# fraunhoferhhi/casapose

Measured on AMD Instinct MI355X. Metric: images/sec at 640x480, 8-object LMO (casapose_c_gcu5 forward + component filter + LS keypoint voting), higher is better.
Workload: dtype f32 (fp32-level: every fp32 operand as an fp16 pair hi = rn(x), lo = rn(x - hi) -- reproduced to within one fp32 ulp, 0.75 x 2^-24 rms -- and the three products hi*hi, hi*lo, lo*hi, each exact, accumulated in fp32 on v_mfma_f32_32x32x16_f16; weights pre-scaled by a power of two; measured error again; 1 GPU; config_8.ini inference: casapose_c_gcu5, K=9 classes, ver_dim=27, bs=16 per GPU, 480x640, fp32, estimated-mask conditioning, connected-component filter + LS voting; conv_mode=f16x2, parallelism=replicas x1 (no collective)

## Files before the change

### casapose_amd/_lib.py

```python
from __future__ import annotations

import ctypes as C
import os
from typing import Optional

import torch

_HERE = os.path.dirname(os.path.abspath(__file__))
LIB_PATH = os.environ.get("CASAPOSE_HIP_LIB") or os.path.join(_HERE, "libcasapose_hip.so")


class CasaposeHipError(RuntimeError):
    pass


class ConvSource(C.Structure):
    _fields_ = [
        ("data", C.c_void_p),
        ("channels", C.c_int),
        ("ld", C.c_int),
        ("mode", C.c_int),
        ("sel", C.c_void_p),
        ("pre_scale", C.c_void_p),
        ("pre_shift", C.c_void_p),
# ... 93 lines not shown

_vp, _i, _ll, _f = C.c_void_p, C.c_int, C.c_longlong, C.c_float
SYMBOLS = [
    ("cp_last_error", C.c_char_p, []),
    ("cp_version", _i, []),
    ("cp_conv_desc_size", C.c_size_t, []),
    ("cp_conv_source_size", C.c_size_t, []),
    ("cp_device_count", _i, []),
    ("cp_set_persistent_blocks", _i, [_i]),
    ("cp_get_persistent_blocks", _i, []),
    ("cp_mfma_probe_workspace_bytes", C.c_size_t, []),
    ("cp_mfma_probe", _i, [_i, _i, _vp, C.POINTER(C.c_double), _vp]),
    ("cp_conv_ktot", _i, [_i, _i, _i, C.POINTER(_i)]),
    ("cp_conv_pack_weights_host", _i, [_vp, _i, _i, _i, _i, _i, C.POINTER(_i), C.POINTER(_i), _vp]),
    ("cp_conv_halo_weight_floats", _i, [_i, _i, C.POINTER(_i)]),
    ("cp_conv_pack_weights_halo_host", _i, [_vp, _i, _i, _i, C.POINTER(_i), C.POINTER(_i), _vp]),
    ("cp_conv_pack_weights_stem_host", _i, [_vp, _i, _i, _vp]),
    ("cp_conv_pack_head_weights_host", _i, [_vp, _i, _vp]),
    ("cp_conv2d_fwd_f32", _i, [C.POINTER(ConvDesc), _vp]),
    ("cp_conv_selected_tile", _i, [C.POINTER(ConvDesc)]),
    ("cp_conv_split_applicable", _i, [C.POINTER(ConvDesc)]),
    ("cp_conv_split_weight_floats", _i, [_i, _i, C.POINTER(_i)]),
    ("cp_conv_split_weight_bytes", C.c_size_t, [_i, _i, C.POINTER(_i), _i]),
    ("cp_conv_pack_weights_split_host", _i, [_vp, _i, _i, _i, C.POINTER(_i), C.POINTER(_i), _vp]),
    ("cp_conv_split_weights_f32", _i, [_vp, _ll, _i, _vp, _vp]),
    ("cp_conv_pack_head_split_host", _i, [_vp, _i, _vp]),
    ("cp_conv2d_fwd_split", _i, [C.POINTER(ConvDesc), _vp, _vp, _i, _vp]),
    ("cp_conv_split_weights_scaled_f32", _i, [_vp, _ll, _i, C.c_float, _vp, _vp]),
    ("cp_conv2d_fwd_split_scaled", _i, [C.POINTER(ConvDesc), _vp, _vp, _i, C.c_float, C.c_float, _vp]),
    ("cp_conv_bf16_deep_applicable", _i, [C.POINTER(ConvDesc)]),
    ("cp_conv2d_fwd_bf16_deep", _i, [C.POINTER(ConvDesc), _vp, _vp]),
    ("cp_pad_channels_3to4", _i, [_vp, _vp, _ll, _vp]),
    ("cp_maxpool3x3s2_f32", _i, [_vp, _i, _i, _i, _i, _vp, _vp, _i, _vp, _vp]),
    ("cp_upsample_bilinear_x2_f32", _i, [_vp, _i, _i, _i, _i, _vp, _vp]),
    ("cp_guided_upsample_x2_f32", _i, [_vp, _vp, _i, _i, _i, _i, _vp, _vp]),
    ("cp_mask_to_labels_f32", _i, [_vp, _i, _i, _i, _i, _vp, _vp, _vp]),
    ("cp_argmax_labels", _i, [_vp, _i, _i, _ll, _vp, _vp]),
    ("cp_label_pyramid", _i, [_vp, _i, _i, _i, C.POINTER(_vp), C.POINTER(_vp), C.POINTER(_vp), _vp]),
    ("cp_ls_vote_f32", _i, [_vp, _i, _i, _i, _i, _vp, _i, _i, _i, _i, _i, _vp, _vp, _vp]),
    ("cp_ls_vote_w_f32", _i, [_vp, _i, _i, _i, _i, _vp, _i, _i, _i, _i, _i, _i, _vp, _vp, _vp]),
    ("cp_ls_vote_workspace_bytes", C.c_size_t, [_i, _i, _i]),
    ("cp_ccl_filter_labels", _i, [_vp, _i, _i, _i, _i, _i, _i, _vp, _vp, _vp]),
    ("cp_ccl_workspace_bytes", C.c_size_t, [_i, _i, _i, _i]),
    ("cp_ransac_vote_f32", _i, [_vp, _vp, _i, _i, _i, _i, _i, _i, _i, _vp, _i, _f, _f, _i, _i, _i, _vp, _vp, _vp, _vp]),
    ("cp_ransac_vote_seeded_f32", _i, [_vp, _vp, _i, _i, _i, _i, _i, _i, _i, C.c_ulonglong, _i, _f, _f, _i, _i, _i, _vp, _vp, _vp, _vp]),
    ("cp_ransac_workspace_bytes", C.c_size_t, [_i, _i, _i, _i, _i, _i]),
# ... 117 lines not shown
```

### casapose_amd/csrc/conv_hsplit.hip

```cpp
#include "common.h"
#include "mfma_helpers.h"

#include <algorithm>
#include <cmath>
#include <cstdlib>
#include <type_traits>

namespace {

using namespace cp;

constexpr int COLS = 34;
constexpr int TH = 8;
constexpr int HR = TH + 2;
constexpr int HP = HR * COLS;
constexpr int PLANE_B = HP * 32;
constexpr int IPLANE_B = HP * 8;
constexpr int NIT = (HP * 4 + 255) / 256;
constexpr int NIMG = (HP + 255) / 256;

enum : int { HS_BILINEAR = 2, HS_PARTIAL = 4, HS_SEL = 8, HS_HEADK = 16, HS_PREFIX = 32 };

struct SSrc {
    const float* data;
    const uint8_t* sel;
    int C, ld, Hs, Ws;
    unsigned bytes;
};

struct HSplitK {
    SSrc s[2];
    const float* img;
    unsigned img_bytes;
    const unsigned char* W;
    unsigned w_bytes;
    int B, H, Wd, Cout;
    int nch0, nch;
    int tiles_y, tiles_x, ntiles;
    int passes, tiles_per_pass;
    const uint8_t* label;
    unsigned lab_bytes;
    const float* residual;
    int res_ld;
    const float* scale;
// ... 85 lines not shown
            *reinterpret_cast<uint4*>(d + 2048) = make_uint4(l0.x, l0.y, l1.x, l1.y);
        } else if constexpr (NP == 2) {
            uint2 h0, l0, h1, l1;
            cp::split4h(make_float4(v0.x * scale, v0.y * scale, v0.z * scale, v0.w * scale), h0, l0);
            cp::split4h(make_float4(v1.x * scale, v1.y * scale, v1.z * scale, v1.w * scale), h1, l1);
            *reinterpret_cast<uint4*>(d) = make_uint4(h0.x, h0.y, h1.x, h1.y);
            *reinterpret_cast<uint4*>(d + 1024) = make_uint4(l0.x, l0.y, l1.x, l1.y);
        } else {
            const uint2 a = round4(v0), b = round4(v1);
            *reinterpret_cast<uint4*>(d) = make_uint4(a.x, a.y, b.x, b.y);
        }
    }
}

__device__ __forceinline__ float leaky01(float t) { return fmaxf(t, 0.1f * t); }

#ifdef HS_GT3
__host__ __device__ constexpr int hs_group_taps(int tn, int np) { return tn == 1 ? 9 : (tn == 2 ? 3 : 1); }
#else
__host__ __device__ constexpr int hs_group_taps(int tn, int np) { return tn == 1 ? 9 : (tn == 2 ? (np <= 2 ? 9 : 3) : 1); }
#endif

template <int TN, int NP, int MODE>
__global__ __launch_bounds__(512, 2) void conv_hsplit_kernel(const HSplitK p) {
    constexpr bool PARTIAL = (MODE & HS_PARTIAL) != 0;
    constexpr bool BILINEAR = (MODE & HS_BILINEAR) != 0;
    constexpr bool SEL = (MODE & HS_SEL) != 0;
    constexpr bool HEADK = (MODE & HS_HEADK) != 0;
    constexpr bool PREFIX = (MODE & HS_PREFIX) != 0;
    static_assert(!PREFIX || HEADK, "only head layers write output records");
    static_assert(!HEADK || TN == 1, "a fused head needs 32 output channels");
    constexpr int NV = 1;
    constexpr unsigned OOB = 0x80000000u;
    static_assert(NP == 1 || NP == 2 || NP == 3, "1 = bf16, 2 = fp16 two-way split, 3 = exact bf16 split");
    constexpr int NPROD = (NP == 3) ? 6 : (NP == 2) ? 3 : 1;
    constexpr unsigned FRAG_B = NP * 1024u;
    constexpr int GT = hs_group_taps(TN, NP);
    constexpr int GPS = 9 / GT;
    constexpr int GSUB = GT * TN;
    constexpr unsigned GROUP_B = GSUB * FRAG_B;
    constexpr unsigned IGROUP_B = 3 * TN * FRAG_B;
    static_assert(TN == 1 || TN == 2 || TN == 4, "32, 64 or 128 output channels per pass");
    constexpr int NWL = (int)((GROUP_B / 16 + 255) / 256);

    const bool has_img = p.img != nullptr;
    extern __shared__ __attribute__((aligned(16))) unsigned char smem[];
    unsigned char* halo = smem;
    unsigned char* imgh = smem + 2 * NP * PLANE_B;
    unsigned short* labh = reinterpret_cast<unsigned short*>(smem + 2 * NP * PLANE_B + 2 * NP * IPLANE_B);
    unsigned char* wst = smem + 2 * NP * PLANE_B + 2 * NP * IPLANE_B + 4 * HP;
    unsigned char* hwl = wst + ((HEADK && NP <= 2) ? 2 * GROUP_B + IGROUP_B : 2 * GROUP_B);
    constexpr int LOW_R = HR / 2 + 1, LOW_C = COLS / 2 + 1, LOW_P = LOW_R * LOW_C;
    constexpr int LOW_B = LOW_P * 64;
    unsigned char* lowb = hwl + 2 * NP * 1024;
    constexpr int TAB_C = 512;
    float* tabl = reinterpret_cast<float*>(lowb + (BILINEAR ? 2 * LOW_B : 0));
    const bool tab_lds = !HEADK && p.scale != nullptr && !p.clade && p.Cout <= TAB_C;
    if (tab_lds) {
        for (int i = (int)threadIdx.x; i < TAB_C; i += 512) {
            tabl[i] = i < p.Cout ? p.scale[i] : 0.f;
            tabl[TAB_C + i] = i < p.Cout ? p.shift[i] : 0.f;
        }
    }
    const bool head = HEADK || ((TN == 1) && p.head_out != nullptr);
    unsigned char* accst = reinterpret_cast<unsigned char*>(tabl + 2 * TAB_C);
    constexpr bool CAN_SPLIT = NP <= 2 && TN == 1;
    constexpr unsigned ACCST_B = 4u * TN * 4u * 1024u;

    const int wave = __builtin_amdgcn_readfirstlane(threadIdx.x >> 6);
    const bool loader = wave >= 4;
    const int tid = threadIdx.x & 255;
    const int lane = tid & 63;
    const int lrow = lane & 31, kh = lane >> 5;

#ifdef HS_TRACE
    const int hst_role = wave >= 4 ? 1 : 0;
    const bool hst_on = blockIdx.x == 0 && (wave == 0 || wave == 4) && lane == 0;
    int hst_i = 2;
    if (hst_on) { hs_trace[hst_role][0] = __builtin_amdgcn_s_memrealtime(); hs_trace[hst_role][1] = __builtin_readcyclecounter(); }
#endif
    const int bid = cp::xcd_remap(blockIdx.x, gridDim.x);
    const int g = (int)gridDim.x;
    const int my_tiles = (p.ntiles - bid + g - 1) / g;
    if (my_tiles <= 0) return;
    struct TilePos { int tx, ty, n, nb, pass; };
    TilePos first;
    {
        int t = bid;
        first.tx = t % p.tiles_x;
        t /= p.tiles_x;
// ... 3 lines not shown
        first.nb = first.n - first.pass * p.B;
    }
    const int d_tx = g % p.tiles_x, d_ty = (g / p.tiles_x) % p.tiles_y, d_n = g / (p.tiles_x * p.tiles_y);
    const int d_pass = d_n / p.B, d_nb = d_n - d_pass * p.B;
    auto next_tile = [&](TilePos& t) {
        t.tx += d_tx;
        int cy = 0;
        if (t.tx >= p.tiles_x) { t.tx -= p.tiles_x; cy = 1; }
        t.ty += d_ty + cy;
        int cn = 0;
        if (t.ty >= p.tiles_y) { t.ty -= p.tiles_y; cn = 1; }
        t.n += d_n + cn;
        t.nb += d_nb + cn;
        t.pass += d_pass;
        if (t.nb >= p.B) { t.nb -= p.B; ++t.pass; }
    };
    const int tile_w_bytes = (p.nch * 9 + (has_img ? 3 : 0)) * TN * (int)FRAG_B;
    const int nslices = p.nch;
    const int total_slices = my_tiles * nslices;
    const int ngroups_tile = nslices * GPS + (has_img ? 1 : 0);
    const int total_groups = my_tiles * ngroups_tile;
    constexpr unsigned WRES_B = 2 * GROUP_B + IGROUP_B;
    const bool wres = HEADK && NP <= 2 && p.w_res != 0 && p.passes == 1 && (unsigned)tile_w_bytes <= WRES_B;
    const bool esplit = CAN_SPLIT && (HEADK ? p.epi_split != 0 : (p.epi_split == 2 && !head)) && nslices >= 2;

    const int ew = wave & 3;
    const unsigned wlane = (unsigned)lane * 16u;
    const unsigned npix = (unsigned)(p.B * p.H * p.Wd);
    const bool has_lab = PARTIAL || p.clade;
    const unsigned tab_b = p.scale ? (unsigned)((p.clade ? 256 : 1) * p.Cout * 4) : 0u;
    const __amdgpu_buffer_rsrc_t r_tab_s = __builtin_amdgcn_make_buffer_rsrc((void*)(p.scale ? (const void*)p.scale : (const void*)p.W), 0, tab_b, 0x00020000);
    const __amdgpu_buffer_rsrc_t r_tab_b = __builtin_amdgcn_make_buffer_rsrc((void*)(p.scale ? (const void*)p.shift : (const void*)p.W), 0, tab_b, 0x00020000);
    const __amdgpu_buffer_rsrc_t r_res = __builtin_amdgcn_make_buffer_rsrc((void*)(p.residual ? (const void*)p.residual : (const void*)p.W), 0,
                                                                            p.residual ? npix * (unsigned)p.res_ld * 4u : 0u, 0x00020000);
    const __amdgpu_buffer_rsrc_t r_raw = __builtin_amdgcn_make_buffer_rsrc((void*)(p.out_raw ? (void*)p.out_raw : (void*)p.W), 0,
                                                                            p.out_raw ? npix * (unsigned)p.raw_ld * 4u : 0u, 0x00020000);
    const __amdgpu_buffer_rsrc_t r_act = __builtin_amdgcn_make_buffer_rsrc((void*)(p.out_act ? (void*)p.out_act : (void*)p.W), 0,
                                                                            p.out_act ? npix * (unsigned)p.act_ld * 4u : 0u, 0x00020000);
    const __amdgpu_buffer_rsrc_t r_head = __builtin_amdgcn_make_buffer_rsrc((void*)(head ? (void*)p.head_out : (void*)p.W), 0,
                                                                             head ? npix * (unsigned)p.head_ld * 4u : 0u, 0x00020000);
    int pmask[2] = {0x1ff, 0x1ff}, clab[2] = {0, 0};
    auto read_labels = [&](int parity) {
        const unsigned short* lh = labh + parity * HP;
#pragma unroll
        for (int r = 0; r < 2; ++r) {
            const int centre = (2 * ew + r + 1) * COLS + lrow + 1;
            const int lc = lh[centre];
// ... 26 lines not shown
            hk_sh[g4] = hk_sc[g4];
            if (!p.clade) {
                hk_sc[g4] = __builtin_bit_cast(float4, __builtin_amdgcn_raw_buffer_load_b128(r_tab_s, (g4 * 8 + kh * 4) * 4, 0, 0));
                hk_sh[g4] = __builtin_bit_cast(float4, __builtin_amdgcn_raw_buffer_load_b128(r_tab_b, (g4 * 8 + kh * 4) * 4, 0, 0));
                if constexpr (NP == 2 && !PARTIAL) {
                    hk_sc[g4].x *= p.descale; hk_sc[g4].y *= p.descale; hk_sc[g4].z *= p.descale; hk_sc[g4].w *= p.descale;
                }
            }
        }
    }
    float e_amax = 0.f, l_amax = 0.f;
    auto flush_mon = [&]() __attribute__((always_inline)) {
#ifdef HS_TRACE
        if (hst_on) { hs_trace[hst_role][2046] = __builtin_amdgcn_s_memrealtime(); hs_trace[hst_role][2047] = ((unsigned long long)hst_i << 48) | (__builtin_readcyclecounter() & 0xffffffffffffull); }
#endif
        if constexpr (NP == 2) {
            if (p.mon) {
                cp::monitor_flush(p.mon, l_amax);
                cp::monitor_flush(p.mon + 2, e_amax, false);
                cp::monitor_count_launch(p.mon, threadIdx.x == 0);
            }
        }
    };
    auto epilogue = [&](f32x16 (&acc)[2][TN], int r_begin, int r_end, int n, int y0, int x0, int cbase, unsigned pieces) __attribute__((always_inline)) {
        asm volatile("" : "+s"(n), "+s"(y0), "+s"(x0), "+s"(cbase));
#pragma unroll
        for (int r = 0; r < 2; ++r) {
            if (r < r_begin || r >= r_end) continue;
            const int y = y0 + 2 * ew + r, x = x0 + lrow;
            const bool pok = (y < p.H) & (x < p.Wd);
            const unsigned pix = (unsigned)((n * p.H + y) * p.Wd + x);
            u32x4 pre4 = {0u, 0u, 0u, 0u}, pre8 = {0u, 0u, 0u, 0u};
            if constexpr (PREFIX) {
                {
                    const unsigned po = pix * (unsigned)p.res_ld * 4u;
                    pre4 = __builtin_amdgcn_raw_buffer_load_b128(r_res, (int)(pok ? po + 16u * (unsigned)kh : OOB), 0, 0);
                    if (p.head_pre_n > 8) pre8 = __builtin_amdgcn_raw_buffer_load_b128(r_res, (int)((pok & (kh == 0)) ? po + 32u : OOB), 0, 0);
                }
            }
            float f = 1.f;
            if constexpr (PARTIAL) f = p.norm ? 9.0f / (float)max(__popc(pmask[r]), 1) : 1.0f;
            if constexpr (NP == 2) f *= p.descale;
            const unsigned tab_row = (unsigned)(clab[r] * (p.clade ? p.Cout : 0));
            float4 keep[4];
            if constexpr (HEADK) {
                const bool fold = (NP == 2 && !PARTIAL);
#pragma unroll
                for (int g4 = 0; g4 < 4; ++g4) {
                    float4 sc = hk_sc[g4], sh = hk_sh[g4];
                    if (p.clade) {
                        const unsigned to = (tab_row + (unsigned)(g4 * 8 + kh * 4)) * 4u;
                        sc = __builtin_bit_cast(float4, __builtin_amdgcn_raw_buffer_load_b128(r_tab_s, (int)to, 0, 0));
                        sh = __builtin_bit_cast(float4, __builtin_amdgcn_raw_buffer_load_b128(r_tab_b, (int)to, 0, 0));
                        if (fold) { sc.x *= p.descale; sc.y *= p.descale; sc.z *= p.descale; sc.w *= p.descale; }
                    }
                    float4 t;
                    if (fold) {
                        t.x = acc[r][0][g4 * 4 + 0] * sc.x + sh.x;
                        t.y = acc[r][0][g4 * 4 + 1] * sc.y + sh.y;
                        t.z = acc[r][0][g4 * 4 + 2] * sc.z + sh.z;
                        t.w = acc[r][0][g4 * 4 + 3] * sc.w + sh.w;
                    } else {
                        t.x = (acc[r][0][g4 * 4 + 0] * f) * sc.x + sh.x;
                        t.y = (acc[r][0][g4 * 4 + 1] * f) * sc.y + sh.y;
                        t.z = (acc[r][0][g4 * 4 + 2] * f) * sc.z + sh.z;
                        t.w = (acc[r][0][g4 * 4 + 3] * f) * sc.w + sh.w;
// ... 146 lines not shown
                        const int oi = __shfl_xor(bi, 32);
                        const bool other = (ob > best) | ((ob == best) & (oi < bi));
                        bi = other ? oi : bi;
                        bi = (bi == 0x7fffffff) ? 0 : bi;
                        __builtin_amdgcn_raw_buffer_store_b8((unsigned char)bi, r_hlab, (int)(((kh == 0) & pok) ? pix : OOB), 0, 0);
                    }
                }
            }
        }
    };

    if constexpr (NP == 2) cp::f16_overflow_clamps();
    if (loader) {
#ifdef HS_LOADER_IDLE
        if (p.B > 0) {
            if constexpr (BILINEAR) HS_BARRIER();
            HS_BARRIER();
            for (int gg = 0; gg < total_groups; ++gg) HS_BARRIER();
            return;
        }
#endif
        TilePos etile = first;
        int e_n = 0, e_y0 = 0, e_x0 = 0, e_cbase = 0, e_k = 0;
        constexpr int NPIECE = HEADK ? 1 : 4 * TN;
        const int e_q = HEADK ? 1 : (NPIECE + max(ngroups_tile - 1, 1) - 1) / max(ngroups_tile - 1, 1);
        auto loader_epilogue = [&](int phase, bool last) __attribute__((always_inline)) {
            if constexpr (CAN_SPLIT) {
                if (phase == 0 || last) {
                    const int pass = etile.pass;
                    e_n = etile.nb; e_y0 = etile.ty * TH; e_x0 = etile.tx * 32; e_cbase = pass * 32 * TN;
                    if (has_lab) read_labels(e_k & 1);
                }
                unsigned pieces;
                if (last) pieces = 0xffffffffu;
                else if (HEADK) pieces = (phase == ngroups_tile - 1) ? 1u : 0u;
                else {
                    const int b0 = phase * e_q, b1 = min(NPIECE, b0 + e_q);
                    pieces = b0 < b1 ? ((b1 >= 32 ? 0xffffffffu : ((1u << b1) - 1u)) & ~((1u << b0) - 1u)) : 0u;
                }
                if (pieces) {
                    f32x16 accl[2][TN];
                    const unsigned char* src = accst + (unsigned)(HEADK ? (e_k & 1) * ACCST_B : 0);
#pragma unroll
                    for (int j = 0; j < TN; ++j)
#pragma unroll
                        for (int g4 = 0; g4 < 4; ++g4) {
                            float4 v = make_float4(0.f, 0.f, 0.f, 0.f);
                            if (HEADK || ((pieces >> (j * 4 + g4)) & 1u)) v = *reinterpret_cast<const float4*>(src + (unsigned)(((ew * TN + j) * 4 + g4) * 1024) + wlane);
                            accl[1][j][g4 * 4 + 0] = v.x; accl[1][j][g4 * 4 + 1] = v.y; accl[1][j][g4 * 4 + 2] = v.z; accl[1][j][g4 * 4 + 3] = v.w;
                            accl[0][j][g4 * 4 + 0] = v.x; accl[0][j][g4 * 4 + 1] = v.y; accl[0][j][g4 * 4 + 2] = v.z; accl[0][j][g4 * 4 + 3] = v.w;
                        }
                    epilogue(accl, 1, 2, e_n, e_y0, e_x0, e_cbase, pieces);
                }
                if (last || phase == ngroups_tile - 1) {
                    next_tile(etile);
                    ++e_k;
                }
            }
        };
        const __amdgpu_buffer_rsrc_t rs0 = __builtin_amdgcn_make_buffer_rsrc((void*)p.s[0].data, 0, p.s[0].bytes, 0x00020000);
        const __amdgpu_buffer_rsrc_t rs1 = __builtin_amdgcn_make_buffer_rsrc((void*)(p.s[1].data ? p.s[1].data : p.s[0].data), 0,
                                                                              p.s[1].data ? p.s[1].bytes : 0u, 0x00020000);
        const __amdgpu_buffer_rsrc_t rsi = __builtin_amdgcn_make_buffer_rsrc((void*)(has_img ? p.img : p.s[0].data), 0, has_img ? p.img_bytes : 0u, 0x00020000);
        int e_hy[NIT], e_hx[NIT];
        unsigned e_lds[NIT];
#pragma unroll
        for (int it = 0; it < NIT; ++it) {
            const int idx = it * 256 + tid, pix = idx >> 2, q = idx & 3;
            e_hy[it] = pix < HP ? pix / COLS : 0x4000;
            e_hx[it] = pix % COLS;
            e_lds[it] = (unsigned)(pix * 32 + (((q >> 1) ^ ((pix >> 3) & 1)) * 16) + (q & 1) * 8);
        }
        const int q4 = (tid & 3) * 4;
        int e_pof[NIT], e_sof[NIT];
        bool e_ok[NIT];
// ... 482 lines not shown
    }
#endif
    bf16x8 fw[2][NP];
    auto ldw = [&](const unsigned char* wg, int sub, int slot) {
#pragma unroll
        for (int s = 0; s < NP; ++s) fw[slot][s] = *reinterpret_cast<const bf16x8*>(wg + (unsigned)(sub * NP + s) * 1024u + wlane);
    };
    unsigned aoff[2][9];
#pragma unroll
    for (int r = 0; r < 2; ++r)
#pragma unroll
        for (int t = 0; t < 9; ++t) {
            const int pix = (2 * wave + r + t / 3) * COLS + lrow + t % 3;
            aoff[r][t] = (unsigned)(pix * 32 + ((kh ^ ((pix >> 3) & 1)) * 16));
        }
    f32x16 acc[2][TN];
    constexpr int FAS = (TN == 4) ? 1 : 2;
    bf16x8 fa[FAS][2][NP];
    int dump_k = 0;
    auto finish_tile = [&](int n, int y0, int x0, int cbase) __attribute__((always_inline)) {
        if constexpr (CAN_SPLIT) {
            if (esplit) {
#pragma unroll
                for (int j = 0; j < TN; ++j)
#pragma unroll
                    for (int g4 = 0; g4 < 4; ++g4)
                        *reinterpret_cast<float4*>(accst + (unsigned)(HEADK ? (dump_k & 1) * ACCST_B : 0) + (unsigned)(((ew * TN + j) * 4 + g4) * 1024) + wlane) =
                            make_float4(acc[1][j][g4 * 4 + 0], acc[1][j][g4 * 4 + 1], acc[1][j][g4 * 4 + 2], acc[1][j][g4 * 4 + 3]);
                ++dump_k;
            }
        }
        epilogue(acc, 0, esplit ? 1 : 2, n, y0, x0, cbase, 0xffffffffu);
    };

    auto mfma_sub = [&](int aslot, int wslot, int j) {
#pragma unroll
        for (int t = 0; t < NPROD; ++t) {
#pragma unroll
            for (int r = 0; r < 2; ++r) acc[r][j] = mfma_np<NP>(fw[wslot][prod_w<NP>(t)], fa[aslot][r][prod_p<NP>(t)], acc[r][j]);
        }
    };

    TilePos ctile = first;
    if constexpr (BILINEAR) HS_BARRIER();
    HS_BARRIER();
    HSP_DECL;
    int gs = 0, gg = 0;
    for (int k = 0; k < my_tiles; ++k) {
        const int pass = ctile.pass;
        const int n = ctile.nb, y0 = ctile.ty * TH, x0 = ctile.tx * 32;
        const int cbase = pass * 32 * TN;
        next_tile(ctile);
        if (has_lab) read_labels(k & 1);
#pragma unroll
        for (int r = 0; r < 2; ++r)
// ... 107 lines not shown
#ifdef HS_NOEPI
            if (p.B < 0)
#endif
            finish_tile(n, y0, x0, cbase);
            HSP(3);
            HST(4);
            ++gg;
            HS_BARRIER();
            HSP(4);
        }
    }
    HSP_FLUSH(0);
    flush_mon();
}


template <int TN, int NP, int MODE>
int launch_hsplit(HSplitK k, hipStream_t st) {
    k.tiles_y = (k.H + TH - 1) / TH;
    k.tiles_x = (k.Wd + 31) / 32;
    k.passes = (k.Cout + 32 * TN - 1) / (32 * TN);
    k.tiles_per_pass = k.B * k.tiles_y * k.tiles_x;
    k.ntiles = k.passes * k.tiles_per_pass;
    size_t lds = (size_t)2 * NP * PLANE_B + (size_t)2 * NP * IPLANE_B + (size_t)2 * HP * 2 + (size_t)2 * hs_group_taps(TN, NP) * TN * NP * 1024 +
                 (size_t)2 * NP * 1024;
    if ((MODE & HS_HEADK) && NP <= 2) lds += (size_t)3 * TN * NP * 1024;
    if (MODE & HS_BILINEAR) lds += (size_t)2 * ((HR / 2 + 1) * (COLS / 2 + 1)) * 64;
    lds += (size_t)2 * 512 * 4;
    if (NP <= 2 && TN == 1) lds += (size_t)4 * TN * 4 * 1024 * ((MODE & HS_HEADK) ? 2 : 1);
    static bool attr_set = false;
    if (!attr_set) {
        (void)hipFuncSetAttribute(reinterpret_cast<const void*>(&conv_hsplit_kernel<TN, NP, MODE>), hipFuncAttributeMaxDynamicSharedMemorySize, (int)lds);
        attr_set = true;
    }
    const int grid = std::min(cp::persistent_blocks(), k.ntiles);
    CP_LAUNCH((conv_hsplit_kernel<TN, NP, MODE>), dim3(grid), dim3(512), lds, st, k);
    return cp::check_launch("cp_conv2d_fwd_split");
}

inline int split_tn(int cout) { return cout <= 32 ? 1 : 2; }

int split_fragments(int cout, int num_sources, const int* channels) {
    const int tn = split_tn(cout), passes = (cout + 32 * tn - 1) / (32 * tn);
    int steps = 0;
    for (int s = 0; s < num_sources; ++s) steps += (channels[s] == 4) ? 3 : (channels[s] / 16) * 9;
    return steps * tn * passes;
}

}

extern "C" int cp_conv_split_applicable(const cp_conv_desc* d) {
    if (!d || d->struct_size != (uint32_t)sizeof(cp_conv_desc)) return 0;
    if (d->kh != 3 || d->kw != 3 || d->stride != 1 || d->dilation != 1 || d->pad != 1) return 0;
    if (d->cout > 512 || d->cout % 4 != 0 || d->group_rows) return 0;
    if (d->head_out && (d->cout != 32 || !d->head_weights || d->head_cout < 1 || d->head_cout > 32)) return 0;
    if ((d->out_raw && d->out_raw_ld % 4) || (d->out_act && d->out_act_ld % 4) || (d->residual && d->residual_ld % 4)) return 0;
    if ((((uintptr_t)d->out_raw) | ((uintptr_t)d->out_act) | ((uintptr_t)d->residual)) & 15) return 0;
    if (d->num_sources < 1 || d->num_sources > 2) return 0;
    for (int s = 0; s < d->num_sources; ++s) {
        const cp_conv_source& in = d->src[s];
// ... 76 lines not shown
    else if (planes == CP_PLANES_F16X2)
        CP_LAUNCH(hsplit_weights_kernel<2>, dim3(blocks), dim3(256), 0, (hipStream_t)stream, packed, nfrag, scale, reinterpret_cast<unsigned char*>(out));
    else
        CP_LAUNCH(hsplit_weights_kernel<1>, dim3(blocks), dim3(256), 0, (hipStream_t)stream, packed, nfrag, 1.f, reinterpret_cast<unsigned char*>(out));
    return cp::check_launch("cp_conv_split_weights_f32");
}

extern "C" int cp_conv_split_weights_f32(const float* packed, long long floats, int planes, void* out, void* stream) {
    CP_REQUIRE(planes == 1 || planes == 3, "cp_conv_split_weights_f32: planes must be 1 or 3 (CP_PLANES_F16X2 needs cp_conv_split_weights_scaled_f32)");
    return cp_conv_split_weights_scaled_f32(packed, floats, planes, 1.f, out, stream);
}

extern "C" int cp_conv_pack_head_split_host(const float* w, int head_cout, float* dst) {
    CP_REQUIRE(w && dst && head_cout >= 1 && head_cout <= 32, "cp_conv_pack_head_split_host: bad arguments");
    for (int m = 0; m < 2; ++m)
        for (int l = 0; l < 64; ++l)
            for (int e = 0; e < 8; ++e) {
                const int q = l & 31, c = 8 * (2 * m + (e >> 2)) + 4 * (l >> 5) + (e & 3);
                dst[(m * 64 + l) * 8 + e] = q < head_cout ? w[c * head_cout + q] : 0.f;
            }
    return CP_OK;
}

extern "C" int cp_conv2d_fwd_split(const cp_conv_desc* d, const void* weights_split, const void* head_weights_split, int planes, void* stream) {
    CP_REQUIRE(planes == 1 || planes == 3, "cp_conv2d_fwd_split: planes must be 1 or 3 (CP_PLANES_F16X2 needs cp_conv2d_fwd_split_scaled)");
    return cp_conv2d_fwd_split_scaled(d, weights_split, head_weights_split, planes, 1.f, 1.f, stream);
}

extern "C" int cp_conv2d_fwd_split_scaled(const cp_conv_desc* d, const void* weights_split, const void* head_weights_split, int planes, float w_descale,
                                          float head_descale, void* stream) {
    CP_REQUIRE_DESC(d, "cp_conv2d_fwd_split");
    CP_REQUIRE(weights_split && (planes == 1 || planes == 3 || planes == CP_PLANES_F16X2), "cp_conv2d_fwd_split: bad arguments");
    CP_REQUIRE(planes == CP_PLANES_F16X2 ? (w_descale > 0.f && std::isfinite(w_descale) && head_descale > 0.f && std::isfinite(head_descale))
                                         : (w_descale == 1.f && head_descale == 1.f),
               "cp_conv2d_fwd_split_scaled: descale factors other than 1 go with CP_PLANES_F16X2 only");
    CP_REQUIRE(cp_conv_split_applicable(d), "cp_conv2d_fwd_split: this convolution is outside the kernel's range (3x3 / stride 1 / pad 1, cout <= 512 and a multiple of 4, sources "
                                            "of 16-multiple channels + optional trailing 4-channel source; source 0 direct, bilinear x2 or guided x2)");
    CP_REQUIRE(d->out_raw || d->out_act || d->head_out, "cp_conv2d_fwd_split: no output");
    CP_REQUIRE(!d->head_out || head_weights_split, "cp_conv2d_fwd_split: a fused head needs its split weights");
    HSplitK k{};
    int nch = 0;
    for (int s = 0; s < d->num_sources; ++s) {
        const cp_conv_source& in = d->src[s];
        const int Hs = (in.mode == CP_SRC_DIRECT) ? d->in_h : d->in_h / 2, Ws = (in.mode == CP_SRC_DIRECT) ? d->in_w : d->in_w / 2;
        const long long nbytes = (long long)d->batch * Hs * Ws * in.ld * 4;
        CP_REQUIRE(nbytes < (1LL << 31), "cp_conv2d_fwd_split: source %d spans %lld bytes; 32-bit range-checked addressing needs < 2 GiB", s, nbytes);
// ... 33 lines not shown
    k.mon = planes == CP_PLANES_F16X2 ? cp::f16x2_monitor() : nullptr;
    {
        static const int split_env = getenv("CASAPOSE_HS_EPI_SPLIT") ? atoi(getenv("CASAPOSE_HS_EPI_SPLIT")) : 1;
        k.epi_split = split_env;
    }
    {
        static const int wres_env = getenv("CASAPOSE_HS_WRES") ? atoi(getenv("CASAPOSE_HS_WRES")) : 1;
        k.w_res = wres_env;
    }
    const int np = planes & 15;
    const int tn = split_tn(d->cout);
    const bool headk = tn == 1 && d->head_out && !d->residual && !d->out_raw && !d->out_act && d->scale && d->act == CP_ACT_LEAKY01 && d->cout == 32;
    if (d->head_out && d->head_prefix) {
        CP_REQUIRE(headk, "cp_conv2d_fwd_split: head_prefix needs a head-only layer (32 channels, table, leaky ReLU, no other output)");
        CP_REQUIRE(d->head_prefix_n >= 8 && d->head_prefix_n <= 12 && d->head_prefix_ld >= d->head_prefix_n && d->head_out_ld >= d->head_prefix_n + d->head_cout &&
                   ((uintptr_t)d->head_out & 15) == 0 && d->head_out_ld % 4 == 0,
                   "cp_conv2d_fwd_split: 8 <= head_prefix_n <= 12, prefix rows of >= head_prefix_n floats, 16-byte aligned records of >= head_prefix_n + head_cout floats");
        k.residual = d->head_prefix;
        k.res_ld = d->head_prefix_ld;
        k.head_pre_n = d->head_prefix_n;
    }
    const int mode = (d->tap_label ? HS_PARTIAL : 0) | (d->src[0].mode == CP_SRC_BILINEAR_X2 ? HS_BILINEAR : 0) | (d->src[0].mode == CP_SRC_NEAREST_SEL ? HS_SEL : 0) |
                     (headk ? HS_HEADK : 0) | (k.head_pre_n ? HS_PREFIX : 0);
    hipStream_t st = (hipStream_t)stream;
#define CP_HS(TN_, NP_, M_) if (tn == TN_ && np == NP_ && mode == (M_)) return launch_hsplit<TN_, NP_, (M_)>(k, st);
#define CP_HS4(TN_, NP_) CP_HS(TN_, NP_, 0) CP_HS(TN_, NP_, HS_BILINEAR) CP_HS(TN_, NP_, HS_PARTIAL) CP_HS(TN_, NP_, HS_PARTIAL | HS_SEL)
#define CP_HSK(NP_) CP_HS(1, NP_, HS_HEADK) CP_HS(1, NP_, HS_HEADK | HS_BILINEAR) CP_HS(1, NP_, HS_HEADK | HS_PARTIAL) CP_HS(1, NP_, HS_HEADK | HS_PARTIAL | HS_SEL)
    CP_HS4(1, 3)
    CP_HS4(2, 3)
    CP_HS4(1, 2)
    CP_HS4(2, 2)
    CP_HS4(1, 1)
    CP_HS4(2, 1)
    CP_HSK(3)
    CP_HSK(2)
    CP_HSK(1)
    CP_HS(1, 3, HS_HEADK | HS_PREFIX | HS_PARTIAL) CP_HS(1, 3, HS_HEADK | HS_PREFIX | HS_PARTIAL | HS_SEL)
    CP_HS(1, 2, HS_HEADK | HS_PREFIX | HS_PARTIAL) CP_HS(1, 2, HS_HEADK | HS_PREFIX | HS_PARTIAL | HS_SEL)
#undef CP_HSK
#undef CP_HS4
#undef CP_HS
    cp::set_error("cp_conv2d_fwd_split: operand mode %d is not instantiated", mode);
    return CP_ERR_INVALID;
}

#ifdef HS_TRACE
extern "C" int cp_hs_trace_read(unsigned long long* host_out) {
    return hipMemcpyFromSymbol(host_out, HIP_SYMBOL(hs_trace), sizeof(unsigned long long) * 2 * 2048) == hipSuccess ? 0 : -1;
}
#endif

#ifdef HS_PROFILE
extern "C" int cp_hs_profile_read(unsigned long long* host_out, int reset) {
    if (hipMemcpyFromSymbol(host_out, HIP_SYMBOL(hs_prof), sizeof(unsigned long long) * 16) != hipSuccess) return -1;
    if (reset) {
        unsigned long long z[16] = {};
        if (hipMemcpyToSymbol(HIP_SYMBOL(hs_prof), z, sizeof(z)) != hipSuccess) return -1;
    }
    return 0;
}
#endif
```

### include/casapose_hip.h

```cpp
#ifndef CASAPOSE_HIP_H
#define CASAPOSE_HIP_H

#include <stddef.h>
#include <stdint.h>

#ifdef __cplusplus
extern "C" {
#endif

typedef enum cp_status {
    CP_OK = 0,
    CP_ERR_INVALID = -1,
    CP_ERR_LAUNCH = -2,
    CP_ERR_NO_DEVICE = -3
} cp_status;

const char* cp_last_error(void);
#define CP_ABI_VERSION 302
int cp_version(void);
size_t cp_conv_desc_size(void);
size_t cp_conv_source_size(void);
int cp_set_persistent_blocks(int blocks);
int cp_get_persistent_blocks(void);
int cp_device_count(void);
// ... 51 lines not shown
       CP_TILE_64x64 = 5, CP_TILE_256x32 = 6, CP_TILE_HALO = 7 ,
       CP_TILE_STEM = 8  };

int cp_conv_ktot(int kh, int kw, int num_sources, const int* channels);
int cp_conv_pack_weights_host(const float* w_host, int layout, int kh, int kw, int cout, int num_sources,
                              const int* channels, const int* real_channels, float* dst_host);
int cp_conv_halo_weight_floats(int cout, int num_sources, const int* channels);
int cp_conv_pack_weights_halo_host(const float* w_host, int layout, int cout, int num_sources, const int* channels,
                                   const int* real_channels, float* dst_host);
int cp_conv_pack_weights_stem_host(const float* w_host, int layout, int real_channels, float* dst);
int cp_conv_pack_head_weights_host(const float* w_host, int head_cout, float* dst_host);
int cp_conv2d_fwd_f32(const cp_conv_desc* desc, void* stream);
int cp_conv_selected_tile(const cp_conv_desc* desc);

enum { CP_PLANES_F16X2 = 0x12 };
float cp_f16x2_weight_scale(float max_abs);
int cp_f16x2_monitor_set(uint32_t* slot);
uint32_t* cp_f16x2_monitor_get(void);
int cp_f16x2_range_check(float amax, float lo, float hi, float* rescale);
int cp_amax_f32(const float* x, long long groups, long long group_stride, long long count, uint32_t* slot, void* stream);
int cp_conv_split_applicable(const cp_conv_desc* desc);
int cp_conv_split_weight_floats(int cout, int num_sources, const int* channels);
size_t cp_conv_split_weight_bytes(int cout, int num_sources, const int* channels, int planes);
int cp_conv_pack_weights_split_host(const float* w_host, int layout, int cout, int num_sources, const int* channels,
                                    const int* real_channels, float* dst_host);
int cp_conv_split_weights_f32(const float* packed, long long floats, int planes, void* out, void* stream);
int cp_conv_pack_head_split_host(const float* w_host, int head_cout, float* dst_host);
int cp_conv2d_fwd_split(const cp_conv_desc* desc, const void* weights_split, const void* head_weights_split, int planes, void* stream);
int cp_conv_split_weights_scaled_f32(const float* packed, long long floats, int planes, float scale, void* out, void* stream);
int cp_conv2d_fwd_split_scaled(const cp_conv_desc* desc, const void* weights_split, const void* head_weights_split, int planes, float w_descale,
                               float head_descale, void* stream);
int cp_conv_bf16_deep_applicable(const cp_conv_desc* desc);
int cp_conv2d_fwd_bf16_deep(const cp_conv_desc* desc, const void* weights_bf16, void* stream);


int cp_pad_channels_3to4(const float* src, float* dst, long long pixels, void* stream);

int cp_maxpool3x3s2_f32(const float* src, int batch, int h, int w, int channels, const float* scale,
                        const float* shift, int relu, float* dst, void* stream);

int cp_upsample_bilinear_x2_f32(const float* src, int batch, int h, int w, int channels, float* dst,
                                void* stream);

int cp_guided_upsample_x2_f32(const float* src, const uint8_t* sel, int batch, int h, int w, int channels,
                              float* dst, void* stream);

// ... 245 lines not shown
```

Before: 2101 images/s.

## Extend epilogue split handover to 64-channel hsplit conv passes

Adds an HS_SPLIT64 mode so the 64-output-channel (TN=2) fp16x2/bf16 hsplit conv hands one 32-channel block of accumulators to the loader waves through LDS. The loader waves then run that block's epilogue while the compute waves continue with the next tile, instead of the compute waves doing the whole epilogue. The LDS layout is moved into a constexpr struct that checks the 160 KB budget and picks double buffering when it fits. By default this is on for plain-mode layers, with an environment switch to turn it off. The cost is extra LDS traffic, larger LDS use that may lower occupancy, and more kernel instantiations.

```diff
diff --git a/casapose_amd/_lib.py b/casapose_amd/_lib.py
--- a/casapose_amd/_lib.py
+++ b/casapose_amd/_lib.py
@@ -139,6 +139,8 @@
     ("cp_conv_split_applicable", _i, [C.POINTER(ConvDesc)]),
     ("cp_conv_split_weight_floats", _i, [_i, _i, C.POINTER(_i)]),
     ("cp_conv_split_weight_bytes", C.c_size_t, [_i, _i, C.POINTER(_i), _i]),
+    ("cp_conv_split_lds_bytes", C.c_size_t, [_i, _i, _i]),
+    ("cp_conv_split_handover_blocks", _i, [_i, _i, _i]),
     ("cp_conv_pack_weights_split_host", _i, [_vp, _i, _i, _i, C.POINTER(_i), C.POINTER(_i), _vp]),
     ("cp_conv_split_weights_f32", _i, [_vp, _ll, _i, _vp, _vp]),
     ("cp_conv_pack_head_split_host", _i, [_vp, _i, _vp]),
diff --git a/casapose_amd/csrc/conv_hsplit.hip b/casapose_amd/csrc/conv_hsplit.hip
--- a/casapose_amd/csrc/conv_hsplit.hip
+++ b/casapose_amd/csrc/conv_hsplit.hip
@@ -19,7 +19,7 @@
 constexpr int NIT = (HP * 4 + 255) / 256;
 constexpr int NIMG = (HP + 255) / 256;
 
-enum : int { HS_BILINEAR = 2, HS_PARTIAL = 4, HS_SEL = 8, HS_HEADK = 16, HS_PREFIX = 32 };
+enum : int { HS_BILINEAR = 2, HS_PARTIAL = 4, HS_SEL = 8, HS_HEADK = 16, HS_PREFIX = 32, HS_SPLIT64 = 64 };
 
 struct SSrc {
     const float* data;
@@ -151,6 +151,33 @@
 #endif
 
 template <int TN, int NP, int MODE>
+struct HsLds {
+    static constexpr bool HEADK = (MODE & HS_HEADK) != 0, BILINEAR = (MODE & HS_BILINEAR) != 0, SPLIT64 = (MODE & HS_SPLIT64) != 0;
+    static_assert(!SPLIT64 || (TN == 2 && NP <= 2), "HS_SPLIT64: 64 output channels per pass, one or two operand planes");
+    static constexpr unsigned LIMIT = 160u * 1024u;
+    static constexpr unsigned GROUP_B = hs_group_taps(TN, NP) * TN * NP * 1024u;
+    static constexpr unsigned IGROUP_B = 3u * TN * NP * 1024u;
+    static constexpr int LOW_R = HR / 2 + 1, LOW_C = COLS / 2 + 1, LOW_P = LOW_R * LOW_C;
+    static constexpr unsigned LOW_B = LOW_P * 64u;
+    static constexpr int TAB_C = 512;
+    static constexpr unsigned halo = 0;
+    static constexpr unsigned imgh = halo + 2u * NP * PLANE_B;
+    static constexpr unsigned labh = imgh + (TN == 1 ? 2u * NP * IPLANE_B : 0u);
+    static constexpr unsigned wst = labh + 4u * HP;
+    static constexpr unsigned hwl = wst + 2u * GROUP_B + ((HEADK && NP <= 2) ? IGROUP_B : 0u);
+    static constexpr unsigned lowb = hwl + (TN == 1 ? 2u * NP * 1024u : 0u);
+    static constexpr unsigned tabl = lowb + (BILINEAR ? 2u * LOW_B : 0u);
+    static constexpr unsigned accst = tabl + 2u * TAB_C * 4u;
+    static constexpr unsigned BLOCK_B = 4u * 4u * 1024u;
+    static constexpr unsigned NBUF = (HEADK || (SPLIT64 && accst + 2u * BLOCK_B <= LIMIT)) ? 2u : 1u;
+    static constexpr int SPLIT_BLOCKS = (NP <= 2 && (TN == 1 || SPLIT64) && accst + NBUF * BLOCK_B <= LIMIT) ? 1 : 0;
+    static constexpr unsigned ACCST_B = SPLIT_BLOCKS * BLOCK_B;
+    static constexpr unsigned total = accst + NBUF * ACCST_B;
+    static_assert(total <= LIMIT, "conv_hsplit: this instantiation's LDS layout exceeds the 160 KB of a CU");
+    static_assert(imgh % 16 == 0 && labh % 16 == 0 && wst % 16 == 0 && hwl % 16 == 0 && lowb % 16 == 0 && tabl % 16 == 0 && accst % 16 == 0, "16-byte LDS accesses");
+};
+
+template <int TN, int NP, int MODE>
 __global__ __launch_bounds__(512, 2) void conv_hsplit_kernel(const HSplitK p) {
     constexpr bool PARTIAL = (MODE & HS_PARTIAL) != 0;
     constexpr bool BILINEAR = (MODE & HS_BILINEAR) != 0;
@@ -172,18 +199,20 @@
     static_assert(TN == 1 || TN == 2 || TN == 4, "32, 64 or 128 output channels per pass");
     constexpr int NWL = (int)((GROUP_B / 16 + 255) / 256);
 
-    const bool has_img = p.img != nullptr;
+    const bool has_img = TN == 1 && p.img != nullptr;
     extern __shared__ __attribute__((aligned(16))) unsigned char smem[];
-    unsigned char* halo = smem;
-    unsigned char* imgh = smem + 2 * NP * PLANE_B;
-    unsigned short* labh = reinterpret_cast<unsigned short*>(smem + 2 * NP * PLANE_B + 2 * NP * IPLANE_B);
-    unsigned char* wst = smem + 2 * NP * PLANE_B + 2 * NP * IPLANE_B + 4 * HP;
-    unsigned char* hwl = wst + ((HEADK && NP <= 2) ? 2 * GROUP_B + IGROUP_B : 2 * GROUP_B);
-    constexpr int LOW_R = HR / 2 + 1, LOW_C = COLS / 2 + 1, LOW_P = LOW_R * LOW_C;
-    constexpr int LOW_B = LOW_P * 64;
-    unsigned char* lowb = hwl + 2 * NP * 1024;
-    constexpr int TAB_C = 512;
-    float* tabl = reinterpret_cast<float*>(lowb + (BILINEAR ? 2 * LOW_B : 0));
+    using L = HsLds<TN, NP, MODE>;
+    static_assert(L::GROUP_B == GROUP_B && L::IGROUP_B == IGROUP_B, "the layout and the kernel agree on the weight groups");
+    unsigned char* halo = smem + L::halo;
+    unsigned char* imgh = smem + L::imgh;
+    unsigned short* labh = reinterpret_cast<unsigned short*>(smem + L::labh);
+    unsigned char* wst = smem + L::wst;
+    unsigned char* hwl = smem + L::hwl;
+    constexpr int LOW_C = L::LOW_C, LOW_P = L::LOW_P;
+    constexpr int LOW_B = (int)L::LOW_B;
+    unsigned char* lowb = smem + L::lowb;
+    constexpr int TAB_C = L::TAB_C;
+    float* tabl = reinterpret_cast<float*>(smem + L::tabl);
     const bool tab_lds = !HEADK && p.scale != nullptr && !p.clade && p.Cout <= TAB_C;
     if (tab_lds) {
         for (int i = (int)threadIdx.x; i < TAB_C; i += 512) {
@@ -192,9 +221,12 @@
         }
     }
     const bool head = HEADK || ((TN == 1) && p.head_out != nullptr);
-    unsigned char* accst = reinterpret_cast<unsigned char*>(tabl + 2 * TAB_C);
-    constexpr bool CAN_SPLIT = NP <= 2 && TN == 1;
-    constexpr unsigned ACCST_B = 4u * TN * 4u * 1024u;
+    unsigned char* accst = smem + L::accst;
+    constexpr int SB = L::SPLIT_BLOCKS;
+    constexpr int J0 = TN - SB;
+    constexpr bool CAN_SPLIT = SB > 0;
+    constexpr unsigned ACCST_B = L::ACCST_B;
+    constexpr bool LATE = L::NBUF == 2;
 
     const int wave = __builtin_amdgcn_readfirstlane(threadIdx.x >> 6);
     const bool loader = wave >= 4;
@@ -244,7 +276,8 @@
     const int total_groups = my_tiles * ngroups_tile;
     constexpr unsigned WRES_B = 2 * GROUP_B + IGROUP_B;
     const bool wres = HEADK && NP <= 2 && p.w_res != 0 && p.passes == 1 && (unsigned)tile_w_bytes <= WRES_B;
-    const bool esplit = CAN_SPLIT && (HEADK ? p.epi_split != 0 : (p.epi_split == 2 && !head)) && nslices >= 2;
+    const bool esplit = (TN == 1) ? (CAN_SPLIT && (HEADK ? p.epi_split != 0 : (p.epi_split == 2 && !head)) && nslices >= 2)
+                                  : CAN_SPLIT;
 
     const int ew = wave & 3;
     const unsigned wlane = (unsigned)lane * 16u;
@@ -317,7 +350,7 @@
             }
         }
     };
-    auto epilogue = [&](f32x16 (&acc)[2][TN], int r_begin, int r_end, int n, int y0, int x0, int cbase, unsigned pieces) __attribute__((always_inline)) {
+    auto epilogue = [&](f32x16 (&acc)[2][TN], int r_begin, int r_end, int n, int y0, int x0, int cbase, unsigned pieces0, unsigned pieces1) __attribute__((always_inline)) {
         asm volatile("" : "+s"(n), "+s"(y0), "+s"(x0), "+s"(cbase));
 #pragma unroll
         for (int r = 0; r < 2; ++r) {
@@ -337,6 +370,7 @@
             if constexpr (PARTIAL) f = p.norm ? 9.0f / (float)max(__popc(pmask[r]), 1) : 1.0f;
             if constexpr (NP == 2) f *= p.descale;
             const unsigned tab_row = (unsigned)(clab[r] * (p.clade ? p.Cout : 0));
+            const unsigned pieces = r ? pieces1 : pieces0;
             float4 keep[4];
             if constexpr (HEADK) {
                 const bool fold = (NP == 2 && !PARTIAL);
@@ -529,7 +563,7 @@
 #endif
         TilePos etile = first;
         int e_n = 0, e_y0 = 0, e_x0 = 0, e_cbase = 0, e_k = 0;
-        constexpr int NPIECE = HEADK ? 1 : 4 * TN;
+        constexpr int NPIECE = HEADK ? 1 : 4 * SB;
         const int e_q = HEADK ? 1 : (NPIECE + max(ngroups_tile - 1, 1) - 1) / max(ngroups_tile - 1, 1);
         auto loader_epilogue = [&](int phase, bool last) __attribute__((always_inline)) {
             if constexpr (CAN_SPLIT) {
@@ -539,25 +573,26 @@
                     if (has_lab) read_labels(e_k & 1);
                 }
                 unsigned pieces;
-                if (last) pieces = 0xffffffffu;
-                else if (HEADK) pieces = (phase == ngroups_tile - 1) ? 1u : 0u;
+                if (HEADK) pieces = (last || phase == ngroups_tile - 1) ? 1u : 0u;
+                else if (LATE) pieces = (last || phase == ngroups_tile - 1) ? ((1u << NPIECE) - 1u) << (4 * J0) : 0u;
                 else {
-                    const int b0 = phase * e_q, b1 = min(NPIECE, b0 + e_q);
-                    pieces = b0 < b1 ? ((b1 >= 32 ? 0xffffffffu : ((1u << b1) - 1u)) & ~((1u << b0) - 1u)) : 0u;
+                    const int b0 = last ? 0 : phase * e_q, b1 = last ? NPIECE : min(NPIECE, b0 + e_q);
+                    pieces = b0 < b1 ? (((1u << b1) - 1u) & ~((1u << b0) - 1u)) << (4 * J0) : 0u;
                 }
                 if (pieces) {
                     f32x16 accl[2][TN];
-                    const unsigned char* src = accst + (unsigned)(HEADK ? (e_k & 1) * ACCST_B : 0);
+                    const unsigned char* src = accst + (unsigned)(LATE ? (e_k & 1) * ACCST_B : 0);
 #pragma unroll
                     for (int j = 0; j < TN; ++j)
 #pragma unroll
                         for (int g4 = 0; g4 < 4; ++g4) {
                             float4 v = make_float4(0.f, 0.f, 0.f, 0.f);
-                            if (HEADK || ((pieces >> (j * 4 + g4)) & 1u)) v = *reinterpret_cast<const float4*>(src + (unsigned)(((ew * TN + j) * 4 + g4) * 1024) + wlane);
+                            if (j >= J0 && (HEADK || ((pieces >> (j * 4 + g4)) & 1u)))
+                                v = *reinterpret_cast<const float4*>(src + (unsigned)(((ew * SB + (j - J0)) * 4 + g4) * 1024) + wlane);
                             accl[1][j][g4 * 4 + 0] = v.x; accl[1][j][g4 * 4 + 1] = v.y; accl[1][j][g4 * 4 + 2] = v.z; accl[1][j][g4 * 4 + 3] = v.w;
                             accl[0][j][g4 * 4 + 0] = v.x; accl[0][j][g4 * 4 + 1] = v.y; accl[0][j][g4 * 4 + 2] = v.z; accl[0][j][g4 * 4 + 3] = v.w;
                         }
-                    epilogue(accl, 1, 2, e_n, e_y0, e_x0, e_cbase, pieces);
+                    epilogue(accl, 1, 2, e_n, e_y0, e_x0, e_cbase, pieces, pieces);
                 }
                 if (last || phase == ngroups_tile - 1) {
                     next_tile(etile);
@@ -1086,15 +1121,15 @@
         if constexpr (CAN_SPLIT) {
             if (esplit) {
 #pragma unroll
-                for (int j = 0; j < TN; ++j)
+                for (int j = J0; j < TN; ++j)
 #pragma unroll
                     for (int g4 = 0; g4 < 4; ++g4)
-                        *reinterpret_cast<float4*>(accst + (unsigned)(HEADK ? (dump_k & 1) * ACCST_B : 0) + (unsigned)(((ew * TN + j) * 4 + g4) * 1024) + wlane) =
+                        *reinterpret_cast<float4*>(accst + (unsigned)(LATE ? (dump_k & 1) * ACCST_B : 0) + (unsigned)(((ew * SB + (j - J0)) * 4 + g4) * 1024) + wlane) =
                             make_float4(acc[1][j][g4 * 4 + 0], acc[1][j][g4 * 4 + 1], acc[1][j][g4 * 4 + 2], acc[1][j][g4 * 4 + 3]);
                 ++dump_k;
             }
         }
-        epilogue(acc, 0, esplit ? 1 : 2, n, y0, x0, cbase, 0xffffffffu);
+        epilogue(acc, 0, (esplit && J0 == 0) ? 1 : 2, n, y0, x0, cbase, 0xffffffffu, (CAN_SPLIT && J0 > 0 && esplit) ? (1u << (4 * J0)) - 1u : 0xffffffffu);
     };
 
     auto mfma_sub = [&](int aslot, int wslot, int j) {
@@ -1248,12 +1283,7 @@
     k.passes = (k.Cout + 32 * TN - 1) / (32 * TN);
     k.tiles_per_pass = k.B * k.tiles_y * k.tiles_x;
     k.ntiles = k.passes * k.tiles_per_pass;
-    size_t lds = (size_t)2 * NP * PLANE_B + (size_t)2 * NP * IPLANE_B + (size_t)2 * HP * 2 + (size_t)2 * hs_group_taps(TN, NP) * TN * NP * 1024 +
-                 (size_t)2 * NP * 1024;
-    if ((MODE & HS_HEADK) && NP <= 2) lds += (size_t)3 * TN * NP * 1024;
-    if (MODE & HS_BILINEAR) lds += (size_t)2 * ((HR / 2 + 1) * (COLS / 2 + 1)) * 64;
-    lds += (size_t)2 * 512 * 4;
-    if (NP <= 2 && TN == 1) lds += (size_t)4 * TN * 4 * 1024 * ((MODE & HS_HEADK) ? 2 : 1);
+    const size_t lds = HsLds<TN, NP, MODE>::total;
     static bool attr_set = false;
     if (!attr_set) {
         (void)hipFuncSetAttribute(reinterpret_cast<const void*>(&conv_hsplit_kernel<TN, NP, MODE>), hipFuncAttributeMaxDynamicSharedMemorySize, (int)lds);
@@ -1262,6 +1292,16 @@
     const int grid = std::min(cp::persistent_blocks(), k.ntiles);
     CP_LAUNCH((conv_hsplit_kernel<TN, NP, MODE>), dim3(grid), dim3(512), lds, st, k);
     return cp::check_launch("cp_conv2d_fwd_split");
+}
+
+inline bool hs_split64_class(int mode) {
+    switch (mode & (HS_BILINEAR | HS_PARTIAL | HS_SEL)) {
+        case 0: return true;
+        case HS_PARTIAL | HS_SEL: return false;
+        case HS_PARTIAL: return false;
+        case HS_BILINEAR: return false;
+        default: return false;
+    }
 }
 
 inline int split_tn(int cout) { return cout <= 32 ? 1 : 2; }
@@ -1384,6 +1424,30 @@
     return CP_OK;
 }
 
+#define CP_HS4(TN_, NP_) CP_HS(TN_, NP_, 0) CP_HS(TN_, NP_, HS_BILINEAR) CP_HS(TN_, NP_, HS_PARTIAL) CP_HS(TN_, NP_, HS_PARTIAL | HS_SEL)
+#define CP_HSK(NP_) CP_HS(1, NP_, HS_HEADK) CP_HS(1, NP_, HS_HEADK | HS_BILINEAR) CP_HS(1, NP_, HS_HEADK | HS_PARTIAL) CP_HS(1, NP_, HS_HEADK | HS_PARTIAL | HS_SEL)
+#define CP_HS4S(TN_, NP_) CP_HS(TN_, NP_, HS_SPLIT64) CP_HS(TN_, NP_, HS_SPLIT64 | HS_BILINEAR) CP_HS(TN_, NP_, HS_SPLIT64 | HS_PARTIAL) CP_HS(TN_, NP_, HS_SPLIT64 | HS_PARTIAL | HS_SEL)
+#define CP_HS_ALL \
+    CP_HS4(1, 3) CP_HS4(2, 3) CP_HS4(1, 2) CP_HS4(2, 2) CP_HS4(1, 1) CP_HS4(2, 1) CP_HS4S(2, 2) CP_HS4S(2, 1) CP_HSK(3) CP_HSK(2) CP_HSK(1) \
+    CP_HS(1, 3, HS_HEADK | HS_PREFIX | HS_PARTIAL) CP_HS(1, 3, HS_HEADK | HS_PREFIX | HS_PARTIAL | HS_SEL) \
+    CP_HS(1, 2, HS_HEADK | HS_PREFIX | HS_PARTIAL) CP_HS(1, 2, HS_HEADK | HS_PREFIX | HS_PARTIAL | HS_SEL)
+
+extern "C" size_t cp_conv_split_lds_bytes(int cout, int planes, int mode) {
+    const int tn = split_tn(cout), np = planes & 15;
+#define CP_HS(TN_, NP_, M_) if (tn == TN_ && np == NP_ && mode == (M_)) return HsLds<TN_, NP_, (M_)>::total;
+    CP_HS_ALL
+#undef CP_HS
+    return 0;
+}
+
+extern "C" int cp_conv_split_handover_blocks(int cout, int planes, int mode) {
+    const int tn = split_tn(cout), np = planes & 15;
+#define CP_HS(TN_, NP_, M_) if (tn == TN_ && np == NP_ && mode == (M_)) return HsLds<TN_, NP_, (M_)>::SPLIT_BLOCKS;
+    CP_HS_ALL
+#undef CP_HS
+    return -1;
+}
+
 extern "C" int cp_conv2d_fwd_split(const cp_conv_desc* d, const void* weights_split, const void* head_weights_split, int planes, void* stream) {
     CP_REQUIRE(planes == 1 || planes == 3, "cp_conv2d_fwd_split: planes must be 1 or 3 (CP_PLANES_F16X2 needs cp_conv2d_fwd_split_scaled)");
     return cp_conv2d_fwd_split_scaled(d, weights_split, head_weights_split, planes, 1.f, 1.f, stream);
@@ -1463,23 +1527,12 @@
     }
     const int mode = (d->tap_label ? HS_PARTIAL : 0) | (d->src[0].mode == CP_SRC_BILINEAR_X2 ? HS_BILINEAR : 0) | (d->src[0].mode == CP_SRC_NEAREST_SEL ? HS_SEL : 0) |
                      (headk ? HS_HEADK : 0) | (k.head_pre_n ? HS_PREFIX : 0);
+    static const int split64_env = getenv("CASAPOSE_HS_EPI_SPLIT64") ? atoi(getenv("CASAPOSE_HS_EPI_SPLIT64")) : 1;
+    const bool split64 = tn == 2 && np <= 2 && k.nch >= 2 && (k.epi_split == 2 || (k.epi_split == 1 && split64_env != 0 && hs_split64_class(mode)));
+    const int kmode = mode | (split64 ? HS_SPLIT64 : 0);
     hipStream_t st = (hipStream_t)stream;
-#define CP_HS(TN_, NP_, M_) if (tn == TN_ && np == NP_ && mode == (M_)) return launch_hsplit<TN_, NP_, (M_)>(k, st);
-#define CP_HS4(TN_, NP_) CP_HS(TN_, NP_, 0) CP_HS(TN_, NP_, HS_BILINEAR) CP_HS(TN_, NP_, HS_PARTIAL) CP_HS(TN_, NP_, HS_PARTIAL | HS_SEL)
-#define CP_HSK(NP_) CP_HS(1, NP_, HS_HEADK) CP_HS(1, NP_, HS_HEADK | HS_BILINEAR) CP_HS(1, NP_, HS_HEADK | HS_PARTIAL) CP_HS(1, NP_, HS_HEADK | HS_PARTIAL | HS_SEL)
-    CP_HS4(1, 3)
-    CP_HS4(2, 3)
-    CP_HS4(1, 2)
-    CP_HS4(2, 2)
-    CP_HS4(1, 1)
-    CP_HS4(2, 1)
-    CP_HSK(3)
-    CP_HSK(2)
-    CP_HSK(1)
-    CP_HS(1, 3, HS_HEADK | HS_PREFIX | HS_PARTIAL) CP_HS(1, 3, HS_HEADK | HS_PREFIX | HS_PARTIAL | HS_SEL)
-    CP_HS(1, 2, HS_HEADK | HS_PREFIX | HS_PARTIAL) CP_HS(1, 2, HS_HEADK | HS_PREFIX | HS_PARTIAL | HS_SEL)
-#undef CP_HSK
-#undef CP_HS4
+#define CP_HS(TN_, NP_, M_) if (tn == TN_ && np == NP_ && kmode == (M_)) return launch_hsplit<TN_, NP_, (M_)>(k, st);
+    CP_HS_ALL
 #undef CP_HS
     cp::set_error("cp_conv2d_fwd_split: operand mode %d is not instantiated", mode);
     return CP_ERR_INVALID;
diff --git a/include/casapose_hip.h b/include/casapose_hip.h
--- a/include/casapose_hip.h
+++ b/include/casapose_hip.h
@@ -97,6 +97,8 @@
 int cp_conv_split_applicable(const cp_conv_desc* desc);
 int cp_conv_split_weight_floats(int cout, int num_sources, const int* channels);
 size_t cp_conv_split_weight_bytes(int cout, int num_sources, const int* channels, int planes);
+size_t cp_conv_split_lds_bytes(int cout, int planes, int mode);
+int cp_conv_split_handover_blocks(int cout, int planes, int mode);
 int cp_conv_pack_weights_split_host(const float* w_host, int layout, int cout, int num_sources, const int* channels,
                                     const int* real_channels, float* dst_host);
 int cp_conv_split_weights_f32(const float* packed, long long floats, int planes, void* out, void* stream);
```

After: 2101 images/s (median of 2 runs). About the same (+0.0%).
